# biaslab/GaussianProcessNode

Measured on AMD Instinct MI355X. Metric: VMP iterations/sec (sparse-GP node sweep, kin40k-shaped synthetic), higher is better.
Workload: dtype f64

## Files before the change

gaussianprocessnode_amd/csrc/sgp_kernels.hip.h:

```cpp
#pragma once
#include <hip/hip_runtime.h>
#include <stdint.h>
#include <utility>

namespace sgp {

constexpr int TB = 64;
constexpr int PS = 80;
constexpr int KB = 16;
constexpr int MAXD = 32;
constexpr int MAXO = 4;
constexpr int LT = TB + 1;

typedef double d4 __attribute__((ext_vector_type(4)));

struct Params {
    double sigma2;
    double jitter;
    double E_logw;
    double n_override;
    double inv_ell[MAXD];
    double W[MAXO * MAXO];
    double prior_iso;
    double pad[7];
// ... 840 lines not shown
    if (info_reset && blockIdx.x == 0 && blockIdx.y == 0 && blockIdx.z == 0 && threadIdx.x == 0) *info_reset = 0;
    stamp_exit(stamps);
}

__global__ void __launch_bounds__(256) k_assemble_b(const double* __restrict__ bpart, const double* __restrict__ data_scalars,
                                                    double* __restrict__ B, int Mp, int T, int nblk, int d_out, int nscal,
                                                    int64_t* stamps, double* __restrict__ bscratch) {
    sum_b_pairs(bpart, B, bscratch, Mp, T, nblk, d_out, blockIdx.x, gridDim.x);
    if (blockIdx.x == 0)
        for (int e = threadIdx.x; e < nscal; e += 256) B[(size_t)Mp * d_out + e] = data_scalars[e];
    stamp_exit(stamps);
}

__global__ void __launch_bounds__(256) k_unpack_stats(const double* __restrict__ pack, double* __restrict__ stats, int Mp, int T,
                                                      int tail, int tile0, int count) {
    const int ntiles = T * (T + 1) / 2, tid = threadIdx.x;
    if ((int)blockIdx.x == count) {
        for (int e = tid; e < tail; e += 256) stats[(size_t)Mp * Mp + e] = pack[(size_t)ntiles * (TB * TB) + e];
        return;
    }
    const int t = tile0 + (int)blockIdx.x;
    int I, J;
    tile_from_index(t, I, J);
    __shared__ double tile[TB * LT];
    const double* src = pack + (size_t)t * (TB * TB);
    for (int e = tid; e < TB * TB; e += 256) {
        const int j = e >> 6, i = e & 63;
        const double v = src[e];
        stats[(size_t)(J * TB + j) * Mp + I * TB + i] = v;
        tile[i * LT + j] = v;
    }
    if (I == J) return;
    __syncthreads();
    for (int e = tid; e < TB * TB; e += 256) {
        const int i = e >> 6, j = e & 63;
        stats[(size_t)(I * TB + i) * Mp + J * TB + j] = tile[i * LT + j];
    }
}

__global__ void __launch_bounds__(256) k_form_lambda(const double* __restrict__ stats, const double* Lambda0,
                                                     const double* xi0, double* Lam, double* xi, const Params* __restrict__ P,
                                                     int M, int Mp, int d_out, int Q, int Qp, int prior_form, int rev, int64_t* stamps,
                                                     int* __restrict__ info_reset) {
    stamp_enter(stamps);
    if (info_reset && blockIdx.x == 0 && blockIdx.y == 0 && threadIdx.x == 0) *info_reset = 0;
    const int gi = blockIdx.x * TB + (threadIdx.x & 63);
    const int jg = threadIdx.x >> 6;
    const double* Psi2 = stats;
    const double* B = stats + (size_t)Mp * Mp;
    for (int jj = 0; jj < 16; ++jj) {
        int gj = blockIdx.y * TB + jg * 16 + jj;
        double v;
        if (gi < Q && gj < Q) {
            int a = gi / M, i = gi % M, b = gj / M, j = gj % M;
            double prior = (prior_form == 1) ? Lambda0[(size_t)gj * Qp + gi] : (gi == gj ? P->prior_iso : 0.0);
            v = prior + P->W[a + b * d_out] * Psi2[(size_t)j * Mp + i];
        } else v = (gi == gj) ? 1.0 : 0.0;
        if (rev) Lam[(size_t)(Qp - 1 - gj) * Qp + (Qp - 1 - gi)] = v;
        else Lam[(size_t)gj * Qp + gi] = v;
    }
    if (blockIdx.y == 0 && threadIdx.x < TB) {
        double v = 0.0;
        if (gi < Q) {
            int a = gi / M, i = gi % M;
            v = (prior_form == 1) ? xi0[gi] : 0.0;
            for (int e = 0; e < d_out; ++e) v = fma(B[(size_t)e * Mp + i], P->W[e + a * d_out], v);
        }
        xi[gi] = v;
    }
}


template <int SRC>
__device__ __forceinline__ double quad_bcast(double v) {
    constexpr int ctrl = SRC | (SRC << 2) | (SRC << 4) | (SRC << 6);
    int lo = __double2loint(v), hi = __double2hiint(v);
    lo = __builtin_amdgcn_mov_dpp(lo, ctrl, 0xf, 0xf, true);
    hi = __builtin_amdgcn_mov_dpp(hi, ctrl, 0xf, 0xf, true);
    return __hiloint2double(hi, lo);
}

template <int N>
__device__ __forceinline__ double row_bcast(double v) {
    constexpr int ctrl = 0x150 + N;
    int lo = __double2loint(v), hi = __double2hiint(v);
    lo = __builtin_amdgcn_mov_dpp(lo, ctrl, 0xf, 0xf, true);
    hi = __builtin_amdgcn_mov_dpp(hi, ctrl, 0xf, 0xf, true);
    return __hiloint2double(hi, lo);
}

template <typename F, int... Is>
__device__ __forceinline__ void static_for_impl(F&& f, std::integer_sequence<int, Is...>) {
    (f(std::integral_constant<int, Is>{}), ...);
}
template <int N, typename F>
__device__ __forceinline__ void static_for(F&& f) {
    static_for_impl(f, std::make_integer_sequence<int, N>{});
}

__device__ __forceinline__ double rsqrt_nr(double d) {
    double y = __builtin_amdgcn_rsq(d);
    const double h = 0.5 * d;
    y = y * fma(-h * y, y, 1.5);
    y = y * fma(-h * y, y, 1.5);
    return y;
}

constexpr int DPS = 17;
constexpr int DPB = 16 * DPS;
template <class F>
__device__ __forceinline__ void solve16(double (&x)[4], const double* Dp, const double* ri, int q, F&& per_pivot) {
    double dk[16][4];
    static_for<16>([&](auto kc) {
        constexpr int k = decltype(kc)::value, ki = k >> 2;
#pragma unroll
        for (int i = ki; i < 4; ++i) dk[k][i] = Dp[(4 * i + q) * DPS + k];
    });
#pragma unroll
    for (int i = 0; i < 4; ++i) x[i] *= ri[4 * i + q];
    static_for<16>([&](auto kc) {
        constexpr int k = decltype(kc)::value;
        constexpr int kq = k & 3, ki = k >> 2;
        const double v = quad_bcast<kq>(x[ki]);
#pragma unroll
        for (int i = ki; i < 4; ++i) x[i] = fma(-v, dk[k][i], x[i]);
        per_pivot(kc);
    });
}

template <int CHUNKS>
__device__ __forceinline__ void mma_left(d4 (&acc)[4], const double* ap, const double* bp) {
    double av[4 * CHUNKS], bv[4 * CHUNKS];
#pragma unroll
    for (int s4 = 0; s4 < 4 * CHUNKS; ++s4) { av[s4] = ap[4 * s4]; bv[s4] = bp[4 * s4]; }
#pragma unroll
    for (int s4 = 0; s4 < 4 * CHUNKS; ++s4) acc[s4 & 3] = __builtin_amdgcn_mfma_f64_16x16x4f64(av[s4], bv[s4], acc[s4 & 3], 0, 0, 0);
}
__device__ __forceinline__ void mma_left_n(d4 (&acc)[4], const double* ap, const double* bp, int chunks) {
#pragma unroll
    for (int u = 0; u < 4; ++u) acc[u] = (d4){0.0, 0.0, 0.0, 0.0};
    if (chunks == 1) mma_left<1>(acc, ap, bp);
    else if (chunks == 2) mma_left<2>(acc, ap, bp);
    else if (chunks == 3) mma_left<3>(acc, ap, bp);
}
template <class Idle>
__device__ __forceinline__ void potf2_tile(double* S, double* Dp, double* rinv, int* info, int col_base, int n_valid, Idle&& idle) {
    const int tid = threadIdx.x, lane = tid & 63, wave = tid >> 6;
    const int r0 = 16 * wave;
    const int li = lane & 15, lk = lane >> 4;
    const int rr = lane >> 2, q = lane & 3;
#pragma unroll 1
    for (int cb = 0; cb < 4; ++cb) {
        if (cb > 0 && wave > cb) {
            d4 acc[4];
            mma_left_n(acc, S + (r0 + li) * LT + lk , S + (16 * cb + li) * LT + lk , cb);
#pragma unroll
            for (int r = 0; r < 4; ++r)
                S[(r0 + lk + 4 * r) * LT + 16 * cb + li] -= (acc[0][r] + acc[1][r]) + (acc[2][r] + acc[3][r]);
        }
        if (wave == cb) {
            const int pr = lane & 15, pq = lane >> 4;
            double a[4], lo[4];
#pragma unroll
            for (int i = 0; i < 4; ++i) {
                const int c = 4 * i + pq;
                a[i] = (c <= pr) ? S[(r0 + pr) * LT + 16 * cb + c] : S[(r0 + c) * LT + 16 * cb + pr];
                lo[i] = 0.0;
            }
            double dsave = 1.0;
            static_for<16>([&](auto kc) {
                constexpr int k = decltype(kc)::value;
                constexpr int kq = k & 3, ki = k >> 2;
                double y[4];
#pragma unroll
                for (int i = ki; i < 4; ++i) y[i] = row_bcast<k>(a[i]);
                const int src = 4 * (16 * kq + pr);
                const double x = __hiloint2double(__builtin_amdgcn_ds_bpermute(src, __double2hiint(a[ki])),
                                                  __builtin_amdgcn_ds_bpermute(src, __double2loint(a[ki])));
                const double d = __hiloint2double(__builtin_amdgcn_readlane(__double2hiint(a[ki]), 16 * kq + k),
                                                  __builtin_amdgcn_readlane(__double2loint(a[ki]), 16 * kq + k));
                dsave = (lane == k) ? d : dsave;
                const double r = __builtin_amdgcn_rcp(d);
                const double e = fma(-d, r, 1.0);
                const double w = fma(e, e, e);
                const double dinv = fma(r, w, r);
                lo[ki] = (pq == kq && pr >= k) ? x : lo[ki];
#pragma unroll
                for (int i = ki; i < 4; ++i) a[i] = fma(-dinv, x * y[i], a[i]);
            });
            const unsigned long long failed = __ballot(lane < 16 && !(dsave > 0.0));
            if (failed != 0ull && lane == 0) {
                const int bad = __builtin_ctzll(failed);
                if (col_base + 16 * cb + bad < n_valid) atomicCAS(info, 0, col_base + 16 * cb + bad + 1);
            }
            const double ri = rsqrt_nr(dsave);
            if (lane < 16) rinv[16 * cb + lane] = ri;
            __builtin_amdgcn_wave_barrier();
            const double rrow = rinv[16 * cb + pr];
#pragma unroll
            for (int i = 0; i < 4; ++i) {
                const int c = 4 * i + pq;
                const double l = lo[i] * rinv[16 * cb + c];
                S[(r0 + pr) * LT + 16 * cb + c] = l;
                Dp[cb * DPB + pr * DPS + c] = (c < pr) ? l * rrow : 0.0;
            }
        } else {
            idle(2 * cb);
        }
        __syncthreads();
        if (wave > cb) {
            double x[4];
#pragma unroll
            for (int i = 0; i < 4; ++i) x[i] = S[(r0 + rr) * LT + 16 * cb + 4 * i + q];
            solve16(x, Dp + cb * DPB, rinv + 16 * cb, q, [](auto) {});
#pragma unroll
            for (int i = 0; i < 4; ++i) S[(r0 + rr) * LT + 16 * cb + 4 * i + q] = x[i];
            __builtin_amdgcn_wave_barrier();
            const double* dp = S + (r0 + li) * LT + 16 * cb + lk;
            double dv[4];
#pragma unroll
            for (int s4 = 0; s4 < 4; ++s4) dv[s4] = dp[4 * s4];
            d4 g[4];
#pragma unroll
            for (int s4 = 0; s4 < 4; ++s4)
                g[s4] = __builtin_amdgcn_mfma_f64_16x16x4f64(dv[s4], dv[s4], (d4){0.0, 0.0, 0.0, 0.0}, 0, 0, 0);
#pragma unroll
            for (int r = 0; r < 4; ++r)
                S[(r0 + lk + 4 * r) * LT + r0 + li] -= (g[0][r] + g[1][r]) + (g[2][r] + g[3][r]);
        } else {
            if (wave < cb) {
#pragma unroll
                for (int i = 0; i < 4; ++i) S[(r0 + rr) * LT + 16 * cb + 4 * i + q] = 0.0;
            }
            idle(2 * cb + 1);
        }
        __syncthreads();
    }
}

__device__ __forceinline__ void trsm_update(double* X, const double* S, int rb, int cb) {
    const int lane = threadIdx.x & 63;
    const int r0 = 16 * rb;
    const int li = lane & 15, lk = lane >> 4;
    d4 acc[4];
    mma_left_n(acc, X + (r0 + li) * LT + lk, S + (16 * cb + li) * LT + lk, cb);
#pragma unroll
    for (int r = 0; r < 4; ++r)
        X[(r0 + lk + 4 * r) * LT + 16 * cb + li] -= (acc[0][r] + acc[1][r]) + (acc[2][r] + acc[3][r]);
}
__device__ __forceinline__ void trsm_solve(double* X, const double* Dp, const double* rinv, int rb, int cb) {
    const int lane = threadIdx.x & 63;
    const int r0 = 16 * rb;
    const int rr = lane >> 2, q = lane & 3;
    double x[4];
#pragma unroll
    for (int i = 0; i < 4; ++i) x[i] = X[(r0 + rr) * LT + 16 * cb + 4 * i + q];
    solve16(x, Dp + cb * DPB, rinv + 16 * cb, q, [](auto) {});
#pragma unroll
    for (int i = 0; i < 4; ++i) X[(r0 + rr) * LT + 16 * cb + 4 * i + q] = x[i];
}
__device__ __forceinline__ void trsm_interval(double* X, const double* S, const double* Dp, const double* rinv, int rb, int it) {
    if (it >= 2) trsm_update(X, S, rb, it);
    trsm_solve(X, Dp, rinv, rb, it);
    if (it == 0) trsm_update(X, S, rb, 1);
}
__device__ __forceinline__ void syrk_slice(d4& g, const double* X, int R, int C, int c) {
    const int lane = threadIdx.x & 63, li = lane & 15, lk = lane >> 4;
    const double* pa = X + (16 * C + li) * LT + 16 * c + lk;
    const double* pb = X + (16 * R + li) * LT + 16 * c + lk;
    double av[4], bv[4];
#pragma unroll
    for (int k4 = 0; k4 < 4; ++k4) { av[k4] = pa[4 * k4]; bv[k4] = pb[4 * k4]; }
#pragma unroll
    for (int k4 = 0; k4 < 4; ++k4) g = __builtin_amdgcn_mfma_f64_16x16x4f64(av[k4], bv[k4], g, 0, 0, 0);
}
__device__ __forceinline__ void syrk_store(const d4& g, double* __restrict__ Dn, int R, int C) {
    const int lane = threadIdx.x & 63, li = lane & 15, lk = lane >> 4;
#pragma unroll
    for (int r = 0; r < 4; ++r) Dn[(16 * C + lk + 4 * r) * TB + 16 * R + li] = g[r];
}

__device__ __forceinline__ void trtri_tile(const double* S, const double* rinv, double* Wt, double* T) {
    const int tid = threadIdx.x, lane = tid & 63, wave = tid >> 6;
    const int li = lane & 15, lk = lane >> 4;
    const int rr = lane >> 2, q = lane & 3;
    for (int e = tid; e < TB * LT; e += 256) Wt[e] = 0.0;
    __syncthreads();
    {
        const int b0 = 16 * wave;
        double w[4], wo[4];
#pragma unroll
        for (int i = 0; i < 4; ++i) { w[i] = (4 * i + q == rr) ? 1.0 : 0.0; wo[i] = 0.0; }
        double lk_[16][4], rv[16];
        static_for<16>([&](auto kc) {
            constexpr int k = decltype(kc)::value, ki = k >> 2;
            rv[k] = rinv[b0 + k];
#pragma unroll
            for (int i = 0; i <= ki; ++i) lk_[k][i] = S[(b0 + k) * LT + b0 + 4 * i + q];
        });
        static_for<16>([&](auto kc) {
            constexpr int k = 15 - decltype(kc)::value;
            constexpr int kq = k & 3, ki = k >> 2;
            const double v = quad_bcast<kq>(w[ki]) * rv[k];
            if (q == kq) wo[ki] = v;
#pragma unroll
            for (int i = 0; i <= ki; ++i) w[i] = fma(-v, lk_[k][i], w[i]);
        });
#pragma unroll
        for (int i = 0; i < 4; ++i) Wt[(b0 + rr) * LT + b0 + 4 * i + q] = wo[i];
    }
    __syncthreads();
    if (wave & 1) {
        const int rb = 16 * wave, cb = 16 * (wave - 1);
        double* Tw = T + (wave >> 1) * (16 * 17);
        d4 acc = (d4){0.0, 0.0, 0.0, 0.0};
#pragma unroll
        for (int s4 = 0; s4 < 4; ++s4)
            acc = __builtin_amdgcn_mfma_f64_16x16x4f64(S[(rb + li) * LT + cb + 4 * s4 + lk],
                                                       Wt[(cb + 4 * s4 + lk) * LT + cb + li], acc, 0, 0, 0);
#pragma unroll
        for (int r = 0; r < 4; ++r) Tw[(lk + 4 * r) * 17 + li] = acc[r];
        __builtin_amdgcn_wave_barrier();
        acc = (d4){0.0, 0.0, 0.0, 0.0};
#pragma unroll
        for (int s4 = 0; s4 < 4; ++s4)
            acc = __builtin_amdgcn_mfma_f64_16x16x4f64(Wt[(rb + li) * LT + rb + 4 * s4 + lk], Tw[(4 * s4 + lk) * 17 + li],
                                                       acc, 0, 0, 0);
#pragma unroll
        for (int r = 0; r < 4; ++r) Wt[(rb + lk + 4 * r) * LT + cb + li] = -acc[r];
    }
    __syncthreads();
    {
        const int ti = wave >> 1, tj = wave & 1;
        d4 acc = (d4){0.0, 0.0, 0.0, 0.0};
#pragma unroll
        for (int s4 = 0; s4 < 8; ++s4)
            acc = __builtin_amdgcn_mfma_f64_16x16x4f64(S[(32 + 16 * ti + li) * LT + 4 * s4 + lk],
                                                       Wt[(4 * s4 + lk) * LT + 16 * tj + li], acc, 0, 0, 0);
#pragma unroll
        for (int r = 0; r < 4; ++r) T[(16 * ti + lk + 4 * r) * 33 + 16 * tj + li] = acc[r];
        __syncthreads();
        acc = (d4){0.0, 0.0, 0.0, 0.0};
#pragma unroll
        for (int s4 = 0; s4 < 8; ++s4)
            acc = __builtin_amdgcn_mfma_f64_16x16x4f64(Wt[(32 + 16 * ti + li) * LT + 32 + 4 * s4 + lk],
                                                       T[(4 * s4 + lk) * 33 + 16 * tj + li], acc, 0, 0, 0);
#pragma unroll
        for (int r = 0; r < 4; ++r) Wt[(32 + 16 * ti + lk + 4 * r) * LT + 16 * tj + li] = -acc[r];
    }
    __syncthreads();
}

struct TileRegs { double v[16]; };
__device__ __forceinline__ void tile_g2r(TileRegs& t, const double* __restrict__ A, size_t ld, int row0, int col0) {
#pragma unroll
    for (int u = 0; u < 8; ++u) {
        const int e = (threadIdx.x & 255) + 256 * u, c = e >> 5, r = (e & 31) * 2;
        const double2 w = *reinterpret_cast<const double2*>(A + (size_t)(col0 + c) * ld + row0 + r);
        t.v[2 * u] = w.x;
        t.v[2 * u + 1] = w.y;
    }
}
constexpr int LAM_MAX_GROUPS = 8;
constexpr int LAM_MAX_COLS = 64;
constexpr int LAM_FORM_EARLY = 0x80;
struct LamForm {
    const double* stats;
    const double* Lambda0;
    const double* xi0;
    double* xi;
    const Params* P;
    int M, Mp, d_out, Q, prior_form;
    int64_t* stamps;
    const long long* col_words;
    long long col_need;
    unsigned char form_step[LAM_MAX_COLS], col_group[LAM_MAX_COLS];
    int spin_limit;
    int* sync_status;
    int trace_chain;
};
__device__ __forceinline__ double load_agent(const double* p) {
    return __hip_atomic_load((const __attribute__((address_space(1))) double*)p, __ATOMIC_RELAXED, __HIP_MEMORY_SCOPE_AGENT);
}
template <bool DENSE, bool MULTI, bool BYPASS = false>
__device__ __forceinline__ double lambda_entry(const LamForm& f, int gi, int gj, int Qp, double prior_iso, double w00) {
    const bool inside = gi < f.Q && gj < f.Q;
    const int si = inside ? gi : 0, sj = inside ? gj : 0;
    int a = 0, i = si, b = 0, j = sj;
    if constexpr (MULTI) { a = si / f.M; i = si % f.M; b = sj / f.M; j = sj % f.M; }
    double psi;
    if constexpr (BYPASS) psi = load_agent(f.stats + (size_t)j * f.Mp + i); else psi = f.stats[(size_t)j * f.Mp + i];
    const double diag = (gi == gj) ? 1.0 : 0.0;
    double prior, w;
    if constexpr (DENSE) prior = f.Lambda0[(size_t)sj * Qp + si]; else prior = diag * prior_iso;
    if constexpr (MULTI) w = f.P->W[a + b * f.d_out]; else w = w00;
    const double m = inside ? 1.0 : 0.0;
    return fma(m * w, psi, fma(m, prior, (1.0 - m) * diag));
}
template <bool DENSE, bool MULTI, bool BYPASS>
__device__ __forceinline__ void tile_form_r_impl(TileRegs& t, const LamForm& f, int Qp, int row0, int col0) {
    const double prior_iso = BYPASS ? load_agent(&f.P->prior_iso) : f.P->prior_iso, w00 = BYPASS ? load_agent(&f.P->W[0]) : f.P->W[0];
#pragma unroll
    for (int u = 0; u < 16; ++u) {
        const int e = (threadIdx.x & 255) + 256 * (u >> 1), c = e >> 5, r = (e & 31) * 2 + (u & 1);
        t.v[u] = lambda_entry<DENSE, MULTI, BYPASS>(f, Qp - 1 - (row0 + r), Qp - 1 - (col0 + c), Qp, prior_iso, w00);
    }
}
__device__ __forceinline__ void tile_form_r(TileRegs& t, const LamForm& f, int Qp, int row0, int col0, bool bypass = false) {
    const bool dense = f.prior_form == 1, multi = f.d_out > 1;
    if (bypass && !multi) {
        if (dense) tile_form_r_impl<true, false, true>(t, f, Qp, row0, col0); else tile_form_r_impl<false, false, true>(t, f, Qp, row0, col0);
        return;
    }
    if (dense) { if (multi) tile_form_r_impl<true, true, false>(t, f, Qp, row0, col0); else tile_form_r_impl<true, false, false>(t, f, Qp, row0, col0); }
    else       { if (multi) tile_form_r_impl<false, true, false>(t, f, Qp, row0, col0); else tile_form_r_impl<false, false, false>(t, f, Qp, row0, col0); }
}
__device__ __forceinline__ void tile_r2s(double* S, const TileRegs& t) {
#pragma unroll
    for (int u = 0; u < 16; ++u) {
        const int e = (threadIdx.x & 255) + 256 * (u >> 1), c = e >> 5, r = (e & 31) * 2 + (u & 1);
        S[r * LT + c] = t.v[u];
    }
}
__device__ __forceinline__ void tile_g2s(double* S, const double* __restrict__ A, size_t ld, int row0, int col0) {
    TileRegs t;
    tile_g2r(t, A, ld, row0, col0);
    tile_r2s(S, t);
// ... 333 lines not shown
    for (int u = 0; u < 4; ++u) {
        const double2 w = src[u];
        s = fma(w.y, tp[2 * u + 1], fma(w.x, tp[2 * u], s));
    }
    red[part * TB + c] = s;
    __syncthreads();
    if (part != 0) return;
    double a[8];
#pragma unroll
    for (int q = 0; q < 8; ++q) a[q] = red[q * TB + c];
    const double ci = ((a[0] + a[1]) + (a[2] + a[3])) + ((a[4] + a[5]) + (a[6] + a[7]));
    partial[(size_t)(Tn - 1 - i) * ld + ld - 1 - k] = ci;
    muacc[k] = prev + ci;
}

__device__ __forceinline__ void form_xi(const LamForm& form, int ld, int tid, bool bypass = false) {
    const double* B = form.stats + (size_t)form.Mp * form.Mp;
    for (int gi = tid; gi < ld; gi += 256) {
        double v = 0.0;
        if (gi < form.Q) {
            const int aa = gi / form.M, i = gi % form.M;
            v = (form.prior_form == 1) ? form.xi0[gi] : 0.0;
            for (int e = 0; e < form.d_out; ++e) {
                const double* bp = B + (size_t)e * form.Mp + i;
                const double* wp = &form.P->W[e + aa * form.d_out];
                v = fma(bypass ? load_agent(bp) : *bp, bypass ? load_agent(wp) : *wp, v);
            }
        }
        form.xi[gi] = v;
    }
}
__device__ __forceinline__ bool wait_stat_group(const LamForm& f, int g) {
    int late = 0;
    if ((threadIdx.x & 63) == 0) {
        const long long* w = f.col_words + g;
        if (!join_ready(w, f.col_need)) {
            late = 1;
            spin_until(w, f.col_need, f.spin_limit, f.sync_status, SYNC_LATE_COLUMN);
        }
    }
    return __builtin_amdgcn_readfirstlane(late) != 0;
}

__device__ long long g_step_trace[8 * 64];
#ifndef SGP_STEP_TRACE_A
#define SGP_STEP_TRACE_A 1
#endif
#ifdef SGP_STEP_TRACE
#define STEP_TRACE(e) do { if (tv_t && a == SGP_STEP_TRACE_A && b == 0 && tw == 0 && lane == 0 && wave == 0 && j < 8) g_step_trace[j * 64 + (xgroup ? 32 : 0) + (e)] = realtime_ticks(); } while (0)
#else
#define STEP_TRACE(e) do { } while (0)
#endif

constexpr int PSTEP_THREADS = 512;
constexpr int POTRF_TWINS = 2;
__host__ __device__ constexpr int potrf_twins(int Tn, int j) { return (Tn - j >= 2) ? POTRF_TWINS : 0; }
constexpr int POTRF_SCRATCH = 3 * TB * TB + 64 + 64;
constexpr int POTRF_LOGDET = 3 * TB * TB + 64;
__global__ void __launch_bounds__(PSTEP_THREADS) k_potrf_step(double* __restrict__ A, int ld, int j, int Tn, int* __restrict__ info,
                                                    int n_valid, double* __restrict__ scratch, double* __restrict__ Winv,
                                                    double* __restrict__ Sacc, const double* __restrict__ tv_xi,
                                                    double* __restrict__ tv_t, double* __restrict__ mu_acc,
                                                    double* __restrict__ uv_part, LamForm form) {
    __shared__ __attribute__((aligned(16))) double lds[2 * TB * PS];
    __shared__ __attribute__((aligned(16))) double tiles[2 * TB * LT];
    __shared__ double dprep[4 * DPB];
    __shared__ double rinv[TB];
    TraceScope trace((form.trace_chain ? 16 : 40) + j);
    const bool xgroup = threadIdx.x >= 256;
    const int tid = threadIdx.x & 255, lane = tid & 63, wave = tid >> 6, wr = wave >> 1, wc = wave & 1;
    {
        const int npot = (Tn - j) * (Tn - j + 1) / 2 + potrf_twins(Tn, j);
        if ((int)blockIdx.x >= npot) {
            int e = blockIdx.x - npot;
            const int nfin = (j >= 2) ? 2 * (j - 1) : 0;
            const int npre = (j < Tn) ? nfin : 0;
            const int nsig = (Sacc && j >= 2 && j < Tn) ? (j - 1) * j / 2 : 0;
            if (e == nfin + npre + nsig) { tvec_role<8>(A, Winv, tv_xi, tv_t, ld, j - 1, lds); return; }
            if (e > nfin + npre + nsig) { mu_row_tile(Winv, tv_t, mu_acc, uv_part, ld, Tn, j - 2, e - (nfin + npre + nsig) - 1, lds); return; }
            if (xgroup) return;
            if (e < nfin) winv_row_tile(A, Winv, ld, j - 1, e >> 1, e & 1, lds, 2, tiles);
            else if (e < nfin + npre) { e -= nfin; winv_row_tile(A, Winv, ld, j, e >> 1, e & 1, lds, 1); }
            else if (e < nfin + npre + nsig) {
                int I, J;
                tile_from_index(e - nfin - npre, I, J);
                sigma_row_tile(Winv, Sacc, ld, j - 2, I, J, lds, tiles);
            }
            return;
        }
    }
    int a, b, tw = 0;
    {
        const int nown = (Tn - j) * (Tn - j + 1) / 2;
        if ((int)blockIdx.x >= nown) { a = 1; b = 0; tw = blockIdx.x - nown + 1; }
        else tile_from_index(blockIdx.x, a, b);
    }
    const int i0 = (j + a) * TB, k0 = (j + b) * TB, j0 = j * TB;
    double* P0 = lds;
    double* P1 = lds + TB * PS;
    double* S = tiles;
    double* X = tiles + TB * LT;
    Acc4 accX;
    acc_zero(accX);
    const bool panel = (b == 0);
    const bool diag_inv = panel && a == 0 && Winv != nullptr;
    if (xgroup && !(panel && (a != 0 || diag_inv))) return;
    const bool lam = form.stats != nullptr;
    const int fword = lam ? (int)form.form_step[j + b] : 0;
    const int fstep = lam ? (fword & (LAM_FORM_EARLY - 1)) : -1;
    const bool early = (fword & LAM_FORM_EARLY) != 0;
    const bool do_form = lam && (early ? (j == 0 && fstep == 1) : fstep == j);
    const bool late_form = lam && early && j >= 1 && fstep == j + 1;
    const bool load_old = !lam || j >= 2 || (early ? (j == 1 && fstep == 1) : fstep < j);
    const bool xi_duty = lam && j == 0 && blockIdx.x == gridDim.x - 1;
    if (!lam && j == 0 && !panel) return;
    bool bypass = false;
    if (lam && form.col_words) {
        if (xi_duty && form.col_group[0] != 0xff) bypass = wait_stat_group(form, form.col_group[0]);
        if (do_form && form.col_group[j + b] != 0xff) bypass = wait_stat_group(form, form.col_group[j + b]) || bypass;
        if (j == 0 && !do_form) {
            if (xi_duty) form_xi(form, ld, tid, bypass);
            return;
        }
        if (blockIdx.x == 0 && !xgroup) trace_mark(200 + j);
    }
    double* Dn_out = scratch + (size_t)(1 + (j & 1)) * TB * TB;
    const double* Dn_in = scratch + (size_t)(2 - (j & 1)) * TB * TB;
    auto move_prev = [&]() {
        const int q0 = (j - 1) * TB;
        for (int e = tid; e < TB * TB; e += 256) A[(size_t)(q0 + (e >> 6)) * ld + q0 + (e & 63)] = scratch[e];
    };
    TileRegs rX, rS, rD;
    if (lam && j == 0) stamp_enter(form.stamps);
    STEP_TRACE(0);
    if (panel) {
        long long* tw_words = reinterpret_cast<long long*>(scratch + 3 * TB * TB);
        if (!xgroup) {
            if (a != 0 || diag_inv) __builtin_amdgcn_s_setprio(3);
            tile_fetch(rS, do_form, load_old, A, form, ld, j0, j0, bypass);
            if (j > 0) {
                tile_g2r(rD, Dn_in, TB, 0, 0);
#pragma unroll
                for (int u = 0; u < 16; ++u) rS.v[u] -= rD.v[u];
            }
            if (xi_duty) form_xi(form, ld, tid, bypass);
            if (a == 0 && tid == 0) tw_words[(j + 1) & 1] = 0;
            tile_r2s(S, rS);
            STEP_TRACE(1);
            __syncthreads();
            STEP_TRACE(2);
            if (a == 0 && j > 0 && !diag_inv) move_prev();
            const bool has_solve = (a != 0) || diag_inv;
            const int ntwf = 1 + potrf_twins(Tn, j);
            int fcount = 0, fR[3], fC[3];
            d4 fg[3];
#pragma unroll
            for (int q = 0; q < 3; ++q) {
                fg[q] = (d4){0.0, 0.0, 0.0, 0.0};
                fR[q] = fC[q] = 0;
                const int t = tw + ntwf * ((wave - 1) + 2 * q);
                if (a == 1 && (wave == 1 || wave == 2) && t < 10) { tile_from_index(t, fR[q], fC[q]); fcount = q + 1; }
            }
            auto fsyrk = [&](int c) {
#pragma unroll
                for (int q = 0; q < 3; ++q)
                    if (q < fcount) syrk_slice(fg[q], X, fR[q], fC[q], c);
            };
            auto idle = [&](int iv) {
                if (!has_solve) return;
                if (wave == 0 && iv >= 4 && iv <= 6) trsm_interval(X, S, dprep, rinv, iv == 4 ? 2 : 3, iv - 4);
                if (iv == 6) { fsyrk(0); fsyrk(1); }
                else if (iv == 7) fsyrk(2);
            };
            potf2_tile(S, dprep, rinv, info, j0, n_valid, idle);
            STEP_TRACE(3);
            if (a == 0 && wave == 3) {
                double lg = -log(rinv[lane]);
                for (int o = 32; o > 0; o >>= 1) lg += __shfl_xor(lg, o);
                if (lane == 0) scratch[POTRF_LOGDET + j] = lg;
            }
            if (fcount > 0) {
                fsyrk(3);
#pragma unroll
                for (int q = 0; q < 3; ++q)
                    if (q < fcount) syrk_store(fg[q], Dn_out, fR[q], fC[q]);
            }
            if (a == 0) {
                if (j == Tn - 1) tile_s2g(S, A, ld, j0, j0);
                else tile_s2g(S, scratch, TB, 0, 0);
            }
            STEP_TRACE(4);
            return;
        }
        const bool below = (a != 0);
        if (below) {
            tile_fetch(rX, do_form, load_old, A, form, ld, i0, j0, bypass);
            if (j > 0) {
                const int p0 = (j - 1) * TB;
                load_panel_n(P0, A, ld, i0, p0, TB, tid);
                load_panel_n(P1, A, ld, k0, p0, TB, tid);
            }
            tile_r2s(X, rX);
        } else {
            for (int e = tid; e < TB * LT; e += 256) X[e] = (e / LT == e % LT) ? 1.0 : 0.0;
        }
        STEP_TRACE(1);
        __syncthreads();
        STEP_TRACE(2);
        if (below && tw > 0 && tid == 0)
            __hip_atomic_fetch_add((__attribute__((address_space(1))) long long*)(tw_words + (j & 1)), 1LL, __ATOMIC_RELAXED,
                                   __HIP_MEMORY_SCOPE_AGENT);
        if (!below && j > 0) move_prev();
        {
            const unsigned nslice = (wave == 0) ? 0x0220u : (wave == 1) ? 0x1003u : 0x0202u;
            int done = 0;
#pragma unroll 1
            for (int it = 0; it < 4; ++it) {
                if (below && j > 0) {
                    const int n = (nslice >> (4 * it)) & 15;
                    for (int q = 0; q < n; ++q) {
                        const int sl = done++;
                        const int li = lane & 15, lk = lane >> 4;
                        const double* ap = P0 + (16 * sl + lk) * PS + wr * 32 + li;
                        const double* bp = P1 + (16 * sl + lk) * PS + wc * 32 + li;
#pragma unroll
                        for (int k4 = 0; k4 < 4; ++k4) {
                            const double a0 = ap[0], a1 = ap[16], b0 = bp[0], b1 = bp[16];
                            accX.t[0][0] = __builtin_amdgcn_mfma_f64_16x16x4f64(a0, b0, accX.t[0][0], 0, 0, 0);
                            accX.t[0][1] = __builtin_amdgcn_mfma_f64_16x16x4f64(a0, b1, accX.t[0][1], 0, 0, 0);
                            accX.t[1][0] = __builtin_amdgcn_mfma_f64_16x16x4f64(a1, b0, accX.t[1][0], 0, 0, 0);
                            accX.t[1][1] = __builtin_amdgcn_mfma_f64_16x16x4f64(a1, b1, accX.t[1][1], 0, 0, 0);
                            ap += 4 * PS; bp += 4 * PS;
                        }
                    }
                    if (done == 4) { tile_sub_acc(X, accX, lane, wr, wc); done = 5; }
                }
                STEP_TRACE(3 + 2 * it);
                __syncthreads();
                STEP_TRACE(4 + 2 * it);
            }
        }
        const bool next = (a == 1);
        const int tw_need = (next && tw == 0) ? potrf_twins(Tn, j) : 0;
        bool tw_ready = true;
#pragma unroll 1
        for (int it = 0; it < 4; ++it) {
            if (it == 3 && tw_need > 0 && lane == 0) tw_ready = join_ready(tw_words + (j & 1), tw_need);
            const bool off = (wave == 2 && it == 0) || (wave == 3 && (it == 1 || it == 2));
            if (!off) trsm_interval(X, S, dprep, rinv, wave, it);
            STEP_TRACE(13 + 2 * it);
            __syncthreads();
            STEP_TRACE(14 + 2 * it);
        }
        STEP_TRACE(11);
        if (!below) tile_s2g_t(X, Winv, ld, j0, j0);
        else if (tw == 0) {
            if (tw_need > 0 && lane == 0 && !tw_ready) {
                int it = 0;
                while (!join_ready(tw_words + (j & 1), tw_need)) {
                    if (++it >= (1 << 21)) { atomicMin(info, -1); break; }
                    __builtin_amdgcn_s_sleep(16);
                }
            }
            tile_s2g(X, A, ld, i0, j0);
        }
        STEP_TRACE(12);
        return;
    }
    tile_fetch(rX, do_form, load_old, A, form, ld, i0, k0, bypass);
    if (xi_duty) form_xi(form, ld, tid, bypass);
    if (j > 0) {
        const int p0 = (j - 1) * TB;
        load_panel_n(P0, A, ld, i0, p0, TB, tid);
        if (a != b) load_panel_n(P1, A, ld, k0, p0, TB, tid);
        __syncthreads();
        tile_mma(accX, P0, (a != b) ? P1 : P0, TB, lane, wr, wc);
        __syncthreads();
    }
    tile_r2s(X, rX);
    __syncthreads();
    tile_sub_acc(X, accX, lane, wr, wc);
    __syncthreads();
    if (late_form) {
        bool late = false;
        if (form.col_words && form.col_group[j + b] != 0xff) late = wait_stat_group(form, form.col_group[j + b]);
        tile_form_r(rX, form, ld, i0, k0, late);
        tile_s2g_add(X, rX, A, ld, i0, k0);
        return;
    }
    tile_s2g(X, A, ld, i0, k0);
}

__device__ __forceinline__ void load_v_column(double (&v)[64], const double* __restrict__ Wp, int Qp, int kb, int j) {
    const double2* src = reinterpret_cast<const double2*>(Wp + (size_t)(Qp - 1 - j) * Qp + (Qp - 64 * (kb + 1)));
#pragma unroll
    for (int u = 0; u < 32; ++u) {
        const double2 w = src[u];
        v[63 - 2 * u] = w.x;
        v[62 - 2 * u] = w.y;
    }
}

struct UvArgs {
    const double* Wp;
    const double* t;
    const double* muacc;
    const double* partial;
    double* LR;
    int64_t* stamps;
    const long long* join;
    long long join_need;
    int spin_limit;
    int* sync_status;
};
__global__ void k_join_wait(const long long* w, long long need, int spin_limit, int* sync_status, int bit, int trace_slot) {
    TraceScope trace(trace_slot);
    if (threadIdx.x == 0 && blockIdx.x == 0) spin_until(w, need, spin_limit, sync_status, bit);
}
__global__ void k_join_set(long long* w, long long v) {
    if (threadIdx.x == 0 && blockIdx.x == 0)
        __hip_atomic_store((__attribute__((address_space(1))) long long*)w, v, __ATOMIC_RELAXED, __HIP_MEMORY_SCOPE_AGENT);
}
__device__ __forceinline__ void uv_cols_role(const UvArgs& u, int Qp, int kb, int jb) {
    const int lane = threadIdx.x, j = 64 * jb + lane;
    double* out = u.LR + (size_t)(64 * kb) * Qp + j;
    if (kb > jb) {
#pragma unroll 16
        for (int kk = 0; kk < 64; ++kk) out[(size_t)kk * Qp] = 0.0;
        stamp_exit(u.stamps);
        return;
    }
    double v[64];
    load_v_column(v, u.Wp, Qp, kb, j);
    double T = 0.0;
    for (int b0 = jb; b0 > kb; b0 -= 8) {
        double pv[8];
#pragma unroll
        for (int e = 0; e < 8; ++e) {
            const int b = b0 - e;
            pv[e] = u.partial[(size_t)max(b, kb + 1) * Qp + j] * ((b > kb) ? 1.0 : 0.0);
        }
#pragma unroll
        for (int e = 0; e < 8; ++e) T += pv[e];
    }
    const double pl = u.t[Qp - 1 - (64 * kb + lane)];
    double above = 0.0;
    for (int b0 = 0; b0 < kb; b0 += 8) {
        double x[8];
#pragma unroll
        for (int e = 0; e < 8; ++e) x[e] = u.t[Qp - 1 - (64 * min(b0 + e, kb - 1) + lane)] * ((b0 + e < kb) ? 1.0 : 0.0);
#pragma unroll
        for (int e = 0; e < 8; ++e) above = fma(x[e], x[e], above);
    }
    for (int o = 32; o > 0; o >>= 1) above += __shfl_xor(above, o);
    double inc = pl * pl;
    for (int o = 1; o < 64; o <<= 1) {
        const double up = __shfl_up(inc, o);
        if (lane >= o) inc += up;
    }
    const double before = __shfl_up(inc, 1);
    const double alpha = (1.0 + above) + (lane > 0 ? before : 0.0), an = fma(pl, pl, alpha);
    const double ir = 1.0 / sqrt(alpha * an);
    const double ckl = an * ir, akl = pl * ir;
    auto lane_value = [](double x, int src) {
        return __hiloint2double(__builtin_amdgcn_readlane(__double2hiint(x), src), __builtin_amdgcn_readlane(__double2loint(x), src));
    };
#pragma unroll
    for (int kk = 63; kk >= 0; --kk) {
        out[(size_t)kk * Qp] = fma(lane_value(ckl, kk), v[kk], lane_value(akl, kk) * T);
        T = fma(lane_value(pl, kk), v[kk], T);
    }
    stamp_exit(u.stamps);
}

__global__ void __launch_bounds__(256) k_gemm32(const double* __restrict__ A, const double* __restrict__ B, double* __restrict__ C,
                                                int ld, int Tn, int mode, int s, int rev, double* __restrict__ mu,
                                                double* __restrict__ R, const double* __restrict__ Psi2,
                                                const double* __restrict__ Kinv, double* __restrict__ trace_part, UvArgs uv,
                                                const double* __restrict__ Sacc) {
    __shared__ double As[64 * PS32];
    __shared__ double Bs[64 * PS32];
    __shared__ double tred[4];
    __shared__ double mup[4 * 64], mus[64];
    TraceScope trace(mode == 0 ? (mu ? 5 : 6) : 255);
    if (mode == 0 && uv.Wp) {
        const int ngemm = Tn * (Tn + 1) / 2 * 4;
// ... 2568 lines not shown
```

Before: 4770.

## Software-pipeline LDS loads ahead of MFMA chains in Cholesky panel kernels

```diff
diff --git a/gaussianprocessnode_amd/csrc/sgp_kernels.hip.h b/gaussianprocessnode_amd/csrc/sgp_kernels.hip.h
--- a/gaussianprocessnode_amd/csrc/sgp_kernels.hip.h
+++ b/gaussianprocessnode_amd/csrc/sgp_kernels.hip.h
@@ -1016,11 +1016,15 @@
 #pragma unroll 1
     for (int cb = 0; cb < 4; ++cb) {
         if (cb > 0 && wave > cb) {
+            double so[4];
+#pragma unroll
+            for (int r = 0; r < 4; ++r) so[r] = S[(r0 + lk + 4 * r) * LT + 16 * cb + li];
+            __builtin_amdgcn_sched_barrier(0);
             d4 acc[4];
             mma_left_n(acc, S + (r0 + li) * LT + lk , S + (16 * cb + li) * LT + lk , cb);
 #pragma unroll
             for (int r = 0; r < 4; ++r)
-                S[(r0 + lk + 4 * r) * LT + 16 * cb + li] -= (acc[0][r] + acc[1][r]) + (acc[2][r] + acc[3][r]);
+                S[(r0 + lk + 4 * r) * LT + 16 * cb + li] = so[r] - ((acc[0][r] + acc[1][r]) + (acc[2][r] + acc[3][r]));
         }
         if (wave == cb) {
             const int pr = lane & 15, pq = lane >> 4;
@@ -1106,11 +1110,15 @@
     const int lane = threadIdx.x & 63;
     const int r0 = 16 * rb;
     const int li = lane & 15, lk = lane >> 4;
+    double xo[4];
+#pragma unroll
+    for (int r = 0; r < 4; ++r) xo[r] = X[(r0 + lk + 4 * r) * LT + 16 * cb + li];
+    __builtin_amdgcn_sched_barrier(0);
     d4 acc[4];
     mma_left_n(acc, X + (r0 + li) * LT + lk, S + (16 * cb + li) * LT + lk, cb);
 #pragma unroll
     for (int r = 0; r < 4; ++r)
-        X[(r0 + lk + 4 * r) * LT + 16 * cb + li] -= (acc[0][r] + acc[1][r]) + (acc[2][r] + acc[3][r]);
+        X[(r0 + lk + 4 * r) * LT + 16 * cb + li] = xo[r] - ((acc[0][r] + acc[1][r]) + (acc[2][r] + acc[3][r]));
 }
 __device__ __forceinline__ void trsm_solve(double* X, const double* Dp, const double* rinv, int rb, int cb) {
     const int lane = threadIdx.x & 63;
@@ -1128,15 +1136,16 @@
     trsm_solve(X, Dp, rinv, rb, it);
     if (it == 0) trsm_update(X, S, rb, 1);
 }
-__device__ __forceinline__ void syrk_slice(d4& g, const double* X, int R, int C, int c) {
+struct SyrkOps { double a[4], b[4]; };
+__device__ __forceinline__ void syrk_slice_load(SyrkOps& o, const double* X, int R, int C, int c) {
     const int lane = threadIdx.x & 63, li = lane & 15, lk = lane >> 4;
     const double* pa = X + (16 * C + li) * LT + 16 * c + lk;
     const double* pb = X + (16 * R + li) * LT + 16 * c + lk;
-    double av[4], bv[4];
-#pragma unroll
-    for (int k4 = 0; k4 < 4; ++k4) { av[k4] = pa[4 * k4]; bv[k4] = pb[4 * k4]; }
-#pragma unroll
-    for (int k4 = 0; k4 < 4; ++k4) g = __builtin_amdgcn_mfma_f64_16x16x4f64(av[k4], bv[k4], g, 0, 0, 0);
+#pragma unroll
+    for (int k4 = 0; k4 < 4; ++k4) { o.a[k4] = pa[4 * k4]; o.b[k4] = pb[4 * k4]; }
+}
+__device__ __forceinline__ void syrk_slice_mma(d4& g, const SyrkOps& o, int k4) {
+    g = __builtin_amdgcn_mfma_f64_16x16x4f64(o.a[k4], o.b[k4], g, 0, 0, 0);
 }
 __device__ __forceinline__ void syrk_store(const d4& g, double* __restrict__ Dn, int R, int C) {
     const int lane = threadIdx.x & 63, li = lane & 15, lk = lane >> 4;
@@ -1776,25 +1785,44 @@
             if (a == 0 && j > 0 && !diag_inv) move_prev();
             const bool has_solve = (a != 0) || diag_inv;
             const int ntwf = 1 + potrf_twins(Tn, j);
-            int fcount = 0, fR[3], fC[3];
-            d4 fg[3];
-#pragma unroll
-            for (int q = 0; q < 3; ++q) {
+            static_assert(10 <= 2 * 2 * (1 + POTRF_TWINS), "two tiles of X X^T per wave must cover the ten lower tiles");
+            int fcount = 0, fR[2], fC[2];
+            d4 fg[2];
+#pragma unroll
+            for (int q = 0; q < 2; ++q) {
                 fg[q] = (d4){0.0, 0.0, 0.0, 0.0};
                 fR[q] = fC[q] = 0;
                 const int t = tw + ntwf * ((wave - 1) + 2 * q);
                 if (a == 1 && (wave == 1 || wave == 2) && t < 10) { tile_from_index(t, fR[q], fC[q]); fcount = q + 1; }
             }
-            auto fsyrk = [&](int c) {
-#pragma unroll
-                for (int q = 0; q < 3; ++q)
-                    if (q < fcount) syrk_slice(fg[q], X, fR[q], fC[q], c);
+            fcount = __builtin_amdgcn_readfirstlane(fcount);
+            auto fsyrk = [&](auto ncv, int c0) {
+                constexpr int NC = decltype(ncv)::value;
+                if (fcount == 0) return;
+                SyrkOps o[NC][2];
+#pragma unroll
+                for (int s = 0; s < NC; ++s)
+#pragma unroll
+                    for (int q = 0; q < 2; ++q) syrk_slice_load(o[s][q], X, fR[q], fC[q], c0 + s);
+                __builtin_amdgcn_sched_barrier(0);
+                if (fcount == 2) {
+#pragma unroll
+                    for (int s = 0; s < NC; ++s)
+#pragma unroll
+                        for (int k4 = 0; k4 < 4; ++k4) { syrk_slice_mma(fg[0], o[s][0], k4); syrk_slice_mma(fg[1], o[s][1], k4); }
+                } else {
+#pragma unroll
+                    for (int s = 0; s < NC; ++s)
+#pragma unroll
+                        for (int k4 = 0; k4 < 4; ++k4) syrk_slice_mma(fg[0], o[s][0], k4);
+                }
+                __builtin_amdgcn_sched_barrier(0);
             };
             auto idle = [&](int iv) {
                 if (!has_solve) return;
                 if (wave == 0 && iv >= 4 && iv <= 6) trsm_interval(X, S, dprep, rinv, iv == 4 ? 2 : 3, iv - 4);
-                if (iv == 6) { fsyrk(0); fsyrk(1); }
-                else if (iv == 7) fsyrk(2);
+                if (iv == 6) fsyrk(std::integral_constant<int, 2>{}, 0);
+                else if (iv == 7) fsyrk(std::integral_constant<int, 1>{}, 2);
             };
             potf2_tile(S, dprep, rinv, info, j0, n_valid, idle);
             STEP_TRACE(3);
@@ -1804,9 +1832,9 @@
                 if (lane == 0) scratch[POTRF_LOGDET + j] = lg;
             }
             if (fcount > 0) {
-                fsyrk(3);
-#pragma unroll
-                for (int q = 0; q < 3; ++q)
+                fsyrk(std::integral_constant<int, 1>{}, 3);
+#pragma unroll
+                for (int q = 0; q < 2; ++q)
                     if (q < fcount) syrk_store(fg[q], Dn_out, fR[q], fC[q]);
             }
             if (a == 0) {
@@ -1836,26 +1864,33 @@
                                    __HIP_MEMORY_SCOPE_AGENT);
         if (!below && j > 0) move_prev();
         {
-            const unsigned nslice = (wave == 0) ? 0x0220u : (wave == 1) ? 0x1003u : 0x0202u;
+            const unsigned nslice = (wave == 0) ? 0x1210u : (wave == 1) ? 0x1003u : 0x0103u;
             int done = 0;
 #pragma unroll 1
             for (int it = 0; it < 4; ++it) {
                 if (below && j > 0) {
-                    const int n = (nslice >> (4 * it)) & 15;
-                    for (int q = 0; q < n; ++q) {
-                        const int sl = done++;
+                    const int n = __builtin_amdgcn_readfirstlane((nslice >> (4 * it)) & 15);
+                    if (n > 0) {
                         const int li = lane & 15, lk = lane >> 4;
-                        const double* ap = P0 + (16 * sl + lk) * PS + wr * 32 + li;
-                        const double* bp = P1 + (16 * sl + lk) * PS + wc * 32 + li;
-#pragma unroll
-                        for (int k4 = 0; k4 < 4; ++k4) {
-                            const double a0 = ap[0], a1 = ap[16], b0 = bp[0], b1 = bp[16];
-                            accX.t[0][0] = __builtin_amdgcn_mfma_f64_16x16x4f64(a0, b0, accX.t[0][0], 0, 0, 0);
-                            accX.t[0][1] = __builtin_amdgcn_mfma_f64_16x16x4f64(a0, b1, accX.t[0][1], 0, 0, 0);
-                            accX.t[1][0] = __builtin_amdgcn_mfma_f64_16x16x4f64(a1, b0, accX.t[1][0], 0, 0, 0);
-                            accX.t[1][1] = __builtin_amdgcn_mfma_f64_16x16x4f64(a1, b1, accX.t[1][1], 0, 0, 0);
-                            ap += 4 * PS; bp += 4 * PS;
+                        const double* ap = P0 + (16 * done + lk) * PS + wr * 32 + li;
+                        const double* bp = P1 + (16 * done + lk) * PS + wc * 32 + li;
+                        double a0 = ap[0], a1 = ap[16], b0 = bp[0], b1 = bp[16];
+                        for (int q = 0; q < n; ++q) {
+#pragma unroll
+                            for (int k4 = 0; k4 < 4; ++k4) {
+                                const int adv = (k4 < 3 || q + 1 < n) ? 4 * PS : 0;
+                                ap += adv; bp += adv;
+                                const double na0 = ap[0], na1 = ap[16], nb0 = bp[0], nb1 = bp[16];
+                                __builtin_amdgcn_sched_barrier(0);
+                                accX.t[0][0] = __builtin_amdgcn_mfma_f64_16x16x4f64(a0, b0, accX.t[0][0], 0, 0, 0);
+                                accX.t[0][1] = __builtin_amdgcn_mfma_f64_16x16x4f64(a0, b1, accX.t[0][1], 0, 0, 0);
+                                accX.t[1][0] = __builtin_amdgcn_mfma_f64_16x16x4f64(a1, b0, accX.t[1][0], 0, 0, 0);
+                                accX.t[1][1] = __builtin_amdgcn_mfma_f64_16x16x4f64(a1, b1, accX.t[1][1], 0, 0, 0);
+                                __builtin_amdgcn_sched_barrier(0);
+                                a0 = na0; a1 = na1; b0 = nb0; b1 = nb1;
+                            }
                         }
+                        done += n;
                     }
                     if (done == 4) { tile_sub_acc(X, accX, lane, wr, wc); done = 5; }
                 }
```

New measurement: 4832, median of 6. +1.3%, better.
